# YQChen8/SSF-SLAM

Measured on AMD Instinct MI355X. Metric: LiDAR front-end frames/sec (mask+feature+GN), 64-beam 120k pts, 1/2/4/8 GPUs, higher is better.
Workload: dtype f32 features / f64 mask+solve

## Files before the change

ssf-slam_amd/csrc/mask_common.hpp:

```cpp
#pragma once
#include "ssf_device.hpp"
#include "ssf_internal.hpp"

#include <float.h>
#include <type_traits>

namespace ssf {

#ifndef SSF_MASK_THREADS
#define SSF_MASK_THREADS 768
#endif
constexpr int kMaskThreads = SSF_MASK_THREADS;

#ifdef SSF_MASK_STAMPS
#define SSF_STAMP(slot)                                                                   \
    do {                                                                                  \
        if (threadIdx.x == 0) {                                                           \
            const unsigned long long _t = __builtin_amdgcn_s_memtime();                   \
            out[26 + (slot)] = (double)(_t - stamp0);                                     \
        }                                                                                 \
    } while (0)
#else
#define SSF_STAMP(slot) do { } while (0)
#endif
constexpr int kNW = kMaskThreads / 64;
#ifndef SSF_LLOYD_DEEP
#define SSF_LLOYD_DEEP 2
#endif
constexpr int kLloydDeep = SSF_LLOYD_DEEP;
#ifndef SSF_KPP_DEEP
#define SSF_KPP_DEEP 2
#endif
constexpr int kKppBlocks = 4096;
constexpr double kPi = 3.14159265358979323846;
#ifndef SSF_LLOYD_FULL_PASSES
#define SSF_LLOYD_FULL_PASSES 4
#endif
constexpr int kLloydFullPasses = SSF_LLOYD_FULL_PASSES;
#ifndef SSF_LLOYD_REFULL
#define SSF_LLOYD_REFULL 4
#endif
constexpr int kLloydRefull = SSF_LLOYD_REFULL;
#ifndef SSF_LLOYD_REC_DEEP
#define SSF_LLOYD_REC_DEEP 8
#endif
constexpr int kLloydRecDeep = SSF_LLOYD_REC_DEEP;
constexpr int kLQ = SSF_LLOYD_REC_DEEP * 128;
constexpr int kLloydMax = 300;

SSF_DEV constexpr int up(int i, int j) { return i * 6 - (i * (i - 1)) / 2 + (j - i); }

struct MaskShared {
    double mean[6], tol;
    double tot[28];
    double cen[12], csn[2], cenp[12], csnp[2];
    double x0[6], ktot[16];
    double logdet[2], logw[2];
    double Aq[21], bq[6], cq, C0;
    double lb;
    double C[36], L[36];
    double sums[29];
    double lsum[14];
    double lhist[kLloydMax * 9];
    float lb1[512], lb2[512];
    int64_t c0, c1;
    double dg_cyc, dg_n, dg_lab, dg_wfull, dg_full1;
#ifdef SSF_MASK_STAMPS
    double dg_e[3];
#endif
    double passes;
    int km_iter, em_iter, strict, converged, done, status, label0, bg, bg_pred, lfull;
    double hnk[2], hq[2], hpm[12];
    int hrc[2];
};

template <class T>
SSF_DEV void load_x(const T* __restrict__ P, const T* __restrict__ Fl, int64_t i, double x[6]) {
    x[0] = (double)Fl[3 * i]; x[1] = (double)Fl[3 * i + 1]; x[2] = (double)Fl[3 * i + 2];
    x[3] = (double)P[3 * i];  x[4] = (double)P[3 * i + 1];  x[5] = (double)P[3 * i + 2];
}

typedef __attribute__((address_space(3))) const double LdsDouble;

SSF_DEV const LdsDouble* lds_laundered(const double* p) {
    uint32_t a = (uint32_t)(uintptr_t)p;
    asm volatile("" : "+v"(a));
    return (const LdsDouble*)(uintptr_t)a;
}

template <class T>
SSF_DEV void load_raw(const T* __restrict__ P, const T* __restrict__ Fl, int64_t i, T r[6]) {
    r[0] = Fl[3 * i]; r[1] = Fl[3 * i + 1]; r[2] = Fl[3 * i + 2];
    r[3] = P[3 * i];  r[4] = P[3 * i + 1];  r[5] = P[3 * i + 2];
}

#ifndef SSF_NT_POINTS
#define SSF_NT_POINTS 1
#endif
#if SSF_NT_POINTS
#define SSF_STREAM_LOAD(p) __builtin_nontemporal_load(p)
#else
#define SSF_STREAM_LOAD(p) (*(p))
#endif

template <class T>
SSF_DEV void load_raw_stream(const T* __restrict__ P, const T* __restrict__ Fl, int64_t i, T r[6]) {
    r[0] = SSF_STREAM_LOAD(&Fl[3 * i]); r[1] = SSF_STREAM_LOAD(&Fl[3 * i + 1]); r[2] = SSF_STREAM_LOAD(&Fl[3 * i + 2]);
    r[3] = SSF_STREAM_LOAD(&P[3 * i]);  r[4] = SSF_STREAM_LOAD(&P[3 * i + 1]);  r[5] = SSF_STREAM_LOAD(&P[3 * i + 2]);
}

template <class Ts>
SSF_DEV void load3_off(const Ts* __restrict__ base, uint32_t o, Ts r[3]) {
    const Ts* p = reinterpret_cast<const Ts*>(reinterpret_cast<const char*>(base) + o);
    r[0] = SSF_STREAM_LOAD(&p[0]); r[1] = SSF_STREAM_LOAD(&p[1]); r[2] = SSF_STREAM_LOAD(&p[2]);
}

SSF_DEV double uni(double v) {
    return __hiloint2double(__builtin_amdgcn_readfirstlane(__double2hiint(v)),
                            __builtin_amdgcn_readfirstlane(__double2loint(v)));
}

template <int D, class Ts, class Fn>
SSF_DEV void for_points_deep(const Ts* __restrict__ P, const Ts* __restrict__ Fl, int64_t r0, int64_t r1, Fn&& fn) {
    if (r1 <= r0) return;
    const Ts* Pb = P + 3 * r0;
    const Ts* Fb = Fl + 3 * r0;
    const uint32_t n = (uint32_t)(r1 - r0), T = blockDim.x, last = n - 1;
    constexpr uint32_t S = 3 * sizeof(Ts);
    const uint32_t j0 = threadIdx.x;
    auto load = [&](uint32_t k, Ts r[6]) { load3_off(Fb, k * S, r); load3_off(Pb, k * S, r + 3); };
    Ts buf[D][6];
#pragma unroll
    for (int d = 0; d < D; ++d) load(min(j0 + d * T, last), buf[d]);
    for (uint32_t base = j0; base < n; base += D * T) {
#pragma unroll
        for (int d = 0; d < D; ++d) {
            const uint32_t j = base + d * T;
            double x[6];
#pragma unroll
            for (int k = 0; k < 6; ++k) x[k] = (double)buf[d][k];
            load(min(j + D * T, last), buf[d]);
            fn(r0 + (int64_t)j, x, j < n);
        }
    }
}

template <class Ts, class Fn2, class Fn1>
SSF_DEV void for_point_pairs(const Ts* __restrict__ P, const Ts* __restrict__ Fl, int64_t r0, int64_t r1, Fn2&& fn2,
                             Fn1&& fn1) {
    const Ts* Pb = P + 3 * r0;
    const Ts* Fb = Fl + 3 * r0;
    const uint32_t n = (uint32_t)(r1 - r0), T = blockDim.x, last = n - 1;
    constexpr uint32_t S = 3 * sizeof(Ts);
    uint32_t i = threadIdx.x;
    if (i >= n) return;
    Ts ra[6], rb[6];
    auto load = [&](uint32_t k, Ts r[6]) { load3_off(Fb, k * S, r); load3_off(Pb, k * S, r + 3); };
    load(i, ra);
    load(min(i + T, last), rb);
    for (; i + T < n; i += 2 * T) {
        double xa[6], xb[6];
#pragma unroll
        for (int d = 0; d < 6; ++d) { xa[d] = (double)ra[d]; xb[d] = (double)rb[d]; }
        load(min(i + 2 * T, last), ra);
        load(min(i + 3 * T, last), rb);
        fn2(xa, xb);
    }
    if (i < n) {
        double xa[6];
#pragma unroll
        for (int d = 0; d < 6; ++d) xa[d] = (double)ra[d];
        fn1(xa);
    }
}

}
```

ssf-slam_amd/csrc/mask_lloyd.hpp:

```cpp
#pragma once
#include "mask_exchange.hpp"

namespace ssf {

SSF_DEV uint2* lloyd_rec_base(uint2* rec, int64_t fb, int f) {
    return rec + ((fb + kLloydSpareRecs * (int64_t)f + 1) & ~(int64_t)1);
}
SSF_DEV uint32_t* lloyd_queue_base(uint2* rec, int64_t total, int n_frames, int64_t fb, int f) {
    return reinterpret_cast<uint32_t*>(rec + lloyd_rec_count(total, n_frames)) + fb + kLloydSpareQueue * (int64_t)f;
}

template <class T>
SSF_DEV bool mask_lloyd(MaskCtx<T>& C, const MaskLds& L, uint2* __restrict__ lloyd_rec, int64_t total,
                        int n_frames) {
    MaskShared& S = L.S;
    const int tid = threadIdx.x;
    const T* P = C.P;
    const T* Fl = C.Fl;
    const double (&mean)[6] = C.mean;
    const int64_t n = C.n, r0 = C.X.r0, r1 = C.X.r1;
    if (tid == 0) { S.strict = 0; S.done = 0; S.lfull = 1; S.dg_cyc = S.dg_n = S.dg_lab = S.dg_wfull = S.dg_full1 = 0.0; }
    uint2* __restrict__ LR = lloyd_rec_base(lloyd_rec, C.fb, C.f);
    uint32_t* __restrict__ LQ = lloyd_queue_base(lloyd_rec, total, n_frames, C.fb, C.f);
    for (int it = 0; it < kLloydMax; ++it) {
        if (tid == 0) {
            double* h = S.lhist + 9 * it;
            for (int k = 0; k < 2; ++k) {
                double sn = 0.0;
                for (int d = 0; d < 6; ++d) sn += S.cen[6 * k + d] * S.cen[6 * k + d];
                S.csn[k] = sn;
            }
            for (int d = 0; d < 6; ++d) h[d] = S.cen[6 + d] - S.cen[d];
            h[6] = S.csn[0] - S.csn[1];
            h[7] = sqrt(S.csn[0]) + sqrt(S.csn[1]);
            h[8] = S.csn[0] + S.csn[1];
        }
        __syncthreads();
        if (tid < it) {
            const double* h = S.lhist + 9 * it;
            const double* g = S.lhist + 9 * tid;
            double dw = 0.0;
            for (int d = 0; d < 6; ++d) dw += (h[d] - g[d]) * (h[d] - g[d]);
            S.lb1[tid] = __double2float_ru(2.0 * sqrt(dw) + 2e-13 * (h[7] + g[7]));
            S.lb2[tid] = __double2float_ru(fabs(h[6] - g[6]) + 1e-13 * (h[8] + g[8]));
        }
        __syncthreads();
        const double csn0 = uni(S.csn[0]), csn1 = uni(S.csn[1]);
        double acc[14];
#pragma unroll
        for (int k = 0; k < 14; ++k) acc[k] = 0.0;
        int changed = 0, nlab = 0;
        const bool full = S.lfull != 0;
#ifdef SSF_MASK_STAMPS
        const unsigned long long pass_t0 = __builtin_amdgcn_s_memtime();
#endif
        const bool wrec = it >= kLloydFullPasses - 1;
        auto label = [&](auto wrec_c, int64_t i, const double* x, int lp, bool val) {
            const LdsDouble* cen = lds_laundered(S.cen);
            double v[6], dt0 = 0.0, dt1 = 0.0, vn = 0.0;
#pragma unroll
            for (int d = 0; d < 6; ++d) {
                v[d] = x[d] - mean[d];
                dt0 += v[d] * cen[d]; dt1 += v[d] * cen[6 + d]; vn += v[d] * v[d];
            }
            const double D0 = -2.0 * dt0 + csn0, D1 = -2.0 * dt1 + csn1;
            const int l = D1 < D0 ? 1 : 0;
            double d1 = full ? (double)l : (double)(l - lp), d0 = full ? 1.0 - d1 : -d1;
            d1 = val ? d1 : 0.0; d0 = val ? d0 : 0.0;
            changed += val && (it == 0 || l != lp);
            acc[0] += d0; acc[7] += d1;
#pragma unroll
            for (int d = 0; d < 6; ++d) { acc[1 + d] += d0 * v[d]; acc[8 + d] += d1 * v[d]; }
            const uint32_t gb = __float_as_uint((float)fabs(D0 - D1));
            const uint32_t nvb = (__float_as_uint(__builtin_sqrtf((float)vn)) + 4u + 0x1FFu) & 0x7FFFFE00u;
            if constexpr (decltype(wrec_c)::value) LR[val ? i : n] = make_uint2(gb ? gb - 1u : 0u, nvb | (uint32_t)it | ((uint32_t)l << 31));
        };
        if (full) {
            const double cpn0 = uni(S.csnp[0]), cpn1 = uni(S.csnp[1]);
            auto full_pass = [&](auto wrec_c) {
                for_points_deep<kLloydDeep>(P, Fl, r0, r1, [&](int64_t i, const double* x, bool val) {
                    const LdsDouble* cenp = lds_laundered(S.cenp);
                    double dp0 = 0.0, dp1 = 0.0;
#pragma unroll
                    for (int d = 0; d < 6; ++d) {
                        const double v = x[d] - mean[d];
                        dp0 += v * cenp[d]; dp1 += v * cenp[6 + d];
                    }
                    const int lp = (-2.0 * dp1 + cpn1) < (-2.0 * dp0 + cpn0) ? 1 : 0;
                    label(wrec_c, i, x, lp, val);
                });
            };
            if (wrec) full_pass(std::true_type{});
            else full_pass(std::false_type{});
            nlab = (int)((r1 - r0 - tid + blockDim.x - 1) / blockDim.x);
        } else {
            const int w = __builtin_amdgcn_readfirstlane(tid >> 6), lane = lane_id();
            const int64_t seg = ((r1 - r0 + kNW - 1) / kNW + 127) / 128 * 128;
            const int64_t ws = r0 + (int64_t)w * seg, we = ws + seg < r1 ? ws + seg : r1;
            uint32_t* __restrict__ WQ = LQ + ws;
            const int64_t qspare = n - ws;
            const uint4* __restrict__ LR4 = reinterpret_cast<const uint4*>(LR);
            const int64_t plast = (n - 1) >> 1;
            uint32_t* Q = L.lq + w * kLQ;
            int qc = 0, nl = 0;
            constexpr int D = kLloydRecDeep;
            uint4 buf[D];
#pragma unroll
            for (int d = 0; d < D; ++d) buf[d] = LR4[min((ws >> 1) + d * 64 + lane, plast)];
            for (int64_t base = ws; base < we; base += D * 128) {
#pragma unroll
                for (int d = 0; d < D; ++d) {
                    const int64_t b = base + d * 128;
                    const uint4 q = buf[d];
#pragma unroll
                    for (int h = 0; h < 2; ++h) {
                        const uint32_t gx = h ? q.z : q.x, gy = h ? q.w : q.y;
                        const int64_t i = b + 2 * lane + h;
                        const int tr = (int)(gy & 0x1FFu);
                        const float nv = __uint_as_float(gy & 0x7FFFFE00u);
                        const bool skip = __uint_as_float(gx) > __builtin_fmaf(S.lb1[tr], nv, S.lb2[tr]) * 1.00001f;
                        const bool nd = (i < we) & !skip;
                        const uint64_t m = __ballot(nd);
                        if (nd) Q[nl + __popcll(m & lanemask_lt())] = (uint32_t)i | (gy & 0x80000000u);
                        nl += __popcll(m);
                    }
                    buf[d] = LR4[min(((b + D * 128) >> 1) + lane, plast)];
                }
                __builtin_amdgcn_wave_barrier();
#pragma unroll
                for (int h = 0; h < 2; ++h)
                    WQ[h * 64 + lane < nl ? qc + h * 64 + lane : qspare + lane] = Q[h * 64 + lane];
                for (int k = 128; k < nl; k += 64)
                    if (k + lane < nl) WQ[qc + k + lane] = Q[k + lane];
                __builtin_amdgcn_wave_barrier();
                qc += nl;
                nl = 0;
            }
            __threadfence_block();
            for (int j0 = 0; j0 < qc; j0 += 512) {
                uint32_t e[8];
#pragma unroll
                for (int k = 0; k < 8; ++k) e[k] = WQ[min(j0 + k * 64 + lane, qc - 1)];
                T px[8][6];
#pragma unroll
                for (int k = 0; k < 8; ++k) load_raw(P, Fl, (int64_t)(e[k] & 0x7FFFFFFFu), px[k]);
#pragma unroll
                for (int k = 0; k < 8; ++k) {
                    double x[6];
#pragma unroll
                    for (int d = 0; d < 6; ++d) x[d] = (double)px[k][d];
                    const bool val = j0 + k * 64 + lane < qc;
                    label(std::true_type{}, (int64_t)(e[k] & 0x7FFFFFFFu), x, (int)(e[k] >> 31), val);
                    nlab += val ? 1 : 0;
                }
            }
        }
        block_sum_rs<14>(acc, L.red);
        changed = block_sum_scalar<int>(changed, L.ired);
        nlab = block_sum_scalar<int>(nlab, L.ired);
        if (C.X.G > 1) {
            double v[16];
#pragma unroll
            for (int k = 0; k < 14; ++k) v[k] = acc[k];
            v[14] = (double)changed; v[15] = (double)nlab;
            if (!exchange<16>(C.X, v, L.xtmp, &L.okflag)) return false;
#pragma unroll
            for (int k = 0; k < 14; ++k) acc[k] = v[k];
            changed = (int)v[14]; nlab = (int)v[15];
        }
        if (tid == 0) {
            S.passes += full ? 1.0 + (wrec ? 8.0 / 24.0 : 0.0)
                             : (8.0 * (double)n + 40.0 * (double)nlab) / (24.0 * (double)n);
            S.km_iter = it + 1;
            for (int k = 0; k < 14; ++k) S.lsum[k] = full ? acc[k] : S.lsum[k] + acc[k];
            S.lfull = full ? it < kLloydFullPasses - 1 : nlab * kLloydRefull > n;
#ifdef SSF_MASK_STAMPS
            if (!full) { S.dg_cyc += (double)(__builtin_amdgcn_s_memtime() - pass_t0); S.dg_n += 1.0; S.dg_lab += nlab; }
            else if (it == kLloydFullPasses - 1) S.dg_wfull = (double)(__builtin_amdgcn_s_memtime() - pass_t0);
            else if (it == 1) S.dg_full1 = (double)(__builtin_amdgcn_s_memtime() - pass_t0);
#endif
            for (int k = 0; k < 12; ++k) S.cenp[k] = S.cen[k];
            S.csnp[0] = S.csn[0]; S.csnp[1] = S.csn[1];
            double shift = 0.0;
            for (int k = 0; k < 2; ++k) {
                const double wgt = S.lsum[7 * k];
                double sh = 0.0;
                for (int d = 0; d < 6; ++d) {
                    const double nc = wgt > 0.0 ? S.lsum[7 * k + 1 + d] * (1.0 / wgt) : S.cen[6 * k + d];
                    const double df = nc - S.cen[6 * k + d];
                    sh += df * df;
                    S.cen[6 * k + d] = nc;
                }
                sh = sqrt(sh);
                shift += sh * sh;
            }
            if (changed == 0) { S.strict = 1; S.done = 1; }
            else if (shift <= S.tol) S.done = 1;
        }
        __syncthreads();
        if (S.done) break;
    }
    return true;
}

}
```

ssf-slam_amd/csrc/mask_seed.hpp:

```cpp
#pragma once
#include "mask_exchange.hpp"

namespace ssf {

template <class T>
SSF_DEV bool mask_pass0(MaskCtx<T>& C, const MaskLds& L, const double* __restrict__ draws) {
    MaskShared& S = L.S;
    const int tid = threadIdx.x;
    const T* P = C.P;
    const T* Fl = C.Fl;
    const int64_t n = C.n, r0 = C.X.r0, r1 = C.X.r1;
    double x0[6];
    load_x(P, Fl, 0, x0);
    double a[27];
#pragma unroll
    for (int i = 0; i < 27; ++i) a[i] = 0.0;
    for_points_deep<kLloydDeep>(P, Fl, r0, r1, [&](int64_t, const double* x, bool val) {
        double v[6], vw[6];
#pragma unroll
        for (int d = 0; d < 6; ++d) { v[d] = x[d] - x0[d]; vw[d] = val ? v[d] : 0.0; a[d] += vw[d]; }
#pragma unroll
        for (int r = 0; r < 6; ++r)
#pragma unroll
            for (int c = r; c < 6; ++c) a[6 + up(r, c)] += vw[r] * v[c];
    });
    block_sum_rs<27>(a, L.red);
    if (!exchange<27>(C.X, a, L.xtmp, &L.okflag)) return false;
    if (tid == 0) {
        const double nn = (double)n;
        double m[6];
        double tol = 0.0;
        for (int d = 0; d < 6; ++d) { m[d] = a[d] / nn; S.mean[d] = x0[d] + m[d]; }
        S.tot[0] = nn;
        for (int d = 0; d < 6; ++d) S.tot[1 + d] = a[d] - nn * m[d];
        for (int r = 0; r < 6; ++r)
            for (int c = r; c < 6; ++c) S.tot[7 + up(r, c)] = a[6 + up(r, c)] - nn * m[r] * m[c];
        for (int d = 0; d < 6; ++d) tol += S.tot[7 + up(d, d)] / nn;
        S.tol = tol / 6.0 * 1e-4;
        for (int d = 0; d < 6; ++d) S.x0[d] = x0[d];
        S.ktot[0] = nn;
        for (int r = 0; r < 3; ++r) { S.ktot[1 + r] = a[r] + a[3 + r]; S.ktot[4 + r] = a[3 + r]; }
        for (int r = 0; r < 3; ++r)
            for (int c = 0; c < 3; ++c) {
                const int fr = r, pr = 3 + r, pc = 3 + c;
                const double sfp = a[6 + (fr <= pc ? up(fr, pc) : up(pc, fr))];
                const double spp = a[6 + (pr <= pc ? up(pr, pc) : up(pc, pr))];
                S.ktot[7 + r * 3 + c] = sfp + spp;
            }
        S.c0 = (int64_t)draws[3 * C.f];
        if (S.c0 < 0) S.c0 = 0;
        if (S.c0 >= n) S.c0 = n - 1;
        S.passes = 1;
    }
    __syncthreads();
    return true;
}

template <class T>
SSF_DEV bool mask_kmeanspp(MaskCtx<T>& C, const MaskLds& L, const double* __restrict__ draws) {
    MaskShared& S = L.S;
    const int tid = threadIdx.x;
    const T* P = C.P;
    const T* Fl = C.Fl;
    const double (&mean)[6] = C.mean;
    const int64_t n = C.n, r0 = C.X.r0, r1 = C.X.r1;
    const int f = C.f;
    double c0[6], cn0 = 0.0;
    {
        double x[6];
        load_x(P, Fl, S.c0, x);
        for (int d = 0; d < 6; ++d) { c0[d] = x[d] - mean[d]; cn0 += c0[d] * c0[d]; }
    }
    const int nw = blockDim.x >> 6, w = tid >> 6, lane = lane_id();
    const int64_t nloc = r1 - r0;
    const int64_t seg = (((nloc + nw - 1) / nw) + 63) / 64 * 64;
    const int64_t ws = r0 + (int64_t)w * seg, we = ws + seg < r1 ? ws + seg : r1;
    auto dist0x = [&](const double* x) {
        double dt = 0.0, xs = 0.0;
#pragma unroll
        for (int d = 0; d < 6; ++d) { const double v = x[d] - mean[d]; dt += c0[d] * v; xs += v * v; }
        const double v = (-2.0 * dt + cn0) + xs;
        return v > 0.0 ? v : 0.0;
    };
    auto dist0 = [&](int64_t i) {
        double x[6];
        load_x(P, Fl, i, x);
        return dist0x(x);
    };
    constexpr int kKppDeep = SSF_KPP_DEEP;
    const int64_t wlast = we > ws ? we - 1 : ws;
    const int64_t spw = seg / 64;
    const bool use_blocks = spw * nw <= kKppBlocks;
    double wsum = 0.0;
    T kb[kKppDeep][6];
    if (ws < we) {
#pragma unroll
        for (int k = 0; k < kKppDeep; ++k) load_raw_stream(P, Fl, min(ws + 64 * k + lane, wlast), kb[k]);
    }
    for (int64_t b0 = ws; b0 < we; b0 += 64 * kKppDeep)
#pragma unroll
    for (int k = 0; k < kKppDeep; ++k) {
        const int64_t b = b0 + 64 * k;
        if (b >= we) break;
        const int64_t i = b + lane;
        double x[6];
#pragma unroll
        for (int d = 0; d < 6; ++d) x[d] = (double)kb[k][d];
        load_raw_stream(P, Fl, min(i + 64 * kKppDeep, wlast), kb[k]);
        const double d = i < we ? dist0x(x) : 0.0;
        wsum += d;
        if (use_blocks) {
            double v = d;
#pragma unroll
            for (int o = 1; o < 64; o <<= 1) {
                const double y = __shfl_up(v, o, 64);
                if (lane >= o) v += y;
            }
            if (lane == 63) L.bsum[w * spw + (b - ws) / 64] = v;
        }
    }
    wsum = wave_sum(wsum);
    if (lane == 0) L.red[w] = wsum;
    if (tid == 0) { L.cand[0] = (unsigned long long)n; L.cand[1] = (unsigned long long)n; }
    __syncthreads();
    double pot = 0.0, carry = 0.0;
    for (int k = 0; k < nw; ++k) { if (k == w) carry = pot; pot += L.red[k]; }
    if (C.X.G > 1) {
        double before = 0.0, total = 0.0;
        if (!exchange_prefix(C.X, pot, L.xtmp, &L.okflag, before, total)) return false;
        carry += before;
        pot = total;
    }
    if (tid == 0) S.passes += 1;
    const double t1 = draws[3 * f + 1] * pot, t2 = draws[3 * f + 2] * pot;
    const double wtot = L.red[w];
    bool f1 = carry + wtot < t1 * (1.0 - 1e-9), f2 = carry + wtot < t2 * (1.0 - 1e-9);
    if (use_blocks) {
        int64_t blk1 = -1, blk2 = -1;
        double cb1 = 0.0, cb2 = 0.0;
        if (lane == 0 && !(f1 && f2)) {
            double cr = carry;
            for (int64_t k = 0; ws + 64 * k < we; ++k) {
                const double tot = L.bsum[w * spw + k];
                if (!f1 && blk1 < 0 && cr + tot >= t1) { blk1 = k; cb1 = cr; }
                if (!f2 && blk2 < 0 && cr + tot >= t2) { blk2 = k; cb2 = cr; }
                if ((f1 || blk1 >= 0) && (f2 || blk2 >= 0)) break;
                cr += tot;
            }
        }
        blk1 = __shfl(blk1, 0, 64); blk2 = __shfl(blk2, 0, 64);
        cb1 = __shfl(cb1, 0, 64); cb2 = __shfl(cb2, 0, 64);
#pragma unroll
        for (int j = 0; j < 2; ++j) {
            const int64_t blk = j ? blk2 : blk1;
            if (blk < 0) continue;
            const int64_t b = ws + 64 * blk;
            const int64_t i = b + lane;
            double v = i < we ? dist0(i) : 0.0;
#pragma unroll
            for (int o = 1; o < 64; o <<= 1) {
                const double y = __shfl_up(v, o, 64);
                if (lane >= o) v += y;
            }
            const double incl = (j ? cb2 : cb1) + v;
            const uint64_t mm = __ballot(i < we && incl >= (j ? t2 : t1));
            if (mm && lane == 0) atomicMin(&L.cand[j], (unsigned long long)(b + __ffsll((unsigned long long)mm) - 1));
        }
        f1 = f2 = true;
    }
    for (int64_t b = ws; b < we && !(f1 && f2); b += 64) {
        const int64_t i = b + lane;
        double v = i < we ? dist0(i) : 0.0;
#pragma unroll
        for (int o = 1; o < 64; o <<= 1) {
            const double y = __shfl_up(v, o, 64);
            if (lane >= o) v += y;
        }
        const double incl = carry + v;
        const uint64_t m1 = __ballot(i < we && incl >= t1), m2 = __ballot(i < we && incl >= t2);
        if (!f1 && m1) { f1 = true; if (lane == 0) atomicMin(&L.cand[0], (unsigned long long)(b + __ffsll((unsigned long long)m1) - 1)); }
        if (!f2 && m2) { f2 = true; if (lane == 0) atomicMin(&L.cand[1], (unsigned long long)(b + __ffsll((unsigned long long)m2) - 1)); }
        carry += __shfl(v, 63, 64);
    }
    __syncthreads();
    double cmin[2] = {(double)L.cand[0], (double)L.cand[1]};
    if (!exchange<2, true>(C.X, cmin, L.xtmp, &L.okflag)) return false;
    const int64_t cand[2] = {cmin[0] < (double)n ? (int64_t)cmin[0] : n - 1,
                             cmin[1] < (double)n ? (int64_t)cmin[1] : n - 1};
    double cc[2][6], ccn[2] = {0.0, 0.0};
    for (int j = 0; j < 2; ++j) {
        double x[6];
        load_x(P, Fl, cand[j], x);
        for (int d = 0; d < 6; ++d) { cc[j][d] = x[d] - mean[d]; ccn[j] += cc[j][d] * cc[j][d]; }
    }
    double cp[2] = {0.0, 0.0};
    if (ws < we) {
#pragma unroll
        for (int k = 0; k < kKppDeep; ++k) load_raw_stream(P, Fl, min(ws + 64 * k + lane, wlast), kb[k]);
    }
    for (int64_t b0 = ws; b0 < we; b0 += 64 * kKppDeep)
#pragma unroll
    for (int k = 0; k < kKppDeep; ++k) {
        const int64_t b = b0 + 64 * k;
        if (b >= we) break;
        const int64_t i = b + lane;
        double x[6];
#pragma unroll
        for (int d = 0; d < 6; ++d) x[d] = (double)kb[k][d];
        load_raw_stream(P, Fl, min(i + 64 * kKppDeep, wlast), kb[k]);
        if (i < we) {
            double xs = 0.0, dt0 = 0.0, dt1 = 0.0, dtc = 0.0;
#pragma unroll
            for (int d = 0; d < 6; ++d) {
                const double v = x[d] - mean[d];
                dtc += c0[d] * v; xs += v * v; dt0 += cc[0][d] * v; dt1 += cc[1][d] * v;
            }
            double di = (-2.0 * dtc + cn0) + xs;
            di = di > 0.0 ? di : 0.0;
            double v0 = (-2.0 * dt0 + ccn[0]) + xs, v1 = (-2.0 * dt1 + ccn[1]) + xs;
            v0 = v0 > 0.0 ? v0 : 0.0; v1 = v1 > 0.0 ? v1 : 0.0;
            cp[0] += v0 < di ? v0 : di;
            cp[1] += v1 < di ? v1 : di;
        }
    }
    block_sum<2>(cp, L.red);
    if (!exchange<2>(C.X, cp, L.xtmp, &L.okflag)) return false;
    if (tid == 0) {
        const int best = cp[1] < cp[0] ? 1 : 0;
        S.c1 = cand[best];
        for (int d = 0; d < 6; ++d) { S.cen[d] = c0[d]; S.cen[6 + d] = cc[best][d]; }
        for (int d = 0; d < 12; ++d) S.cenp[d] = 0.0;
        S.csnp[0] = S.csnp[1] = 0.0;
        S.passes += 2;
    }
    __syncthreads();
    return true;
}

}
```

Before: 65600.

## Fuse k-means++ distance prefix into pass0 and first Lloyd step into candidate pass

The per-block prefix sums of distance to the first centre now come from the moments pass (pass0), so k-means++ no longer rereads all points to build them. The final candidate-evaluation sweep also accumulates the Lloyd iteration-0 assignment sums for both candidate centres. It then keeps the winning set and performs the first centroid update, so Lloyd starts at iteration 1. This removes two full streaming passes over the point cloud, at the cost of more registers and a wider reduction (30 values) in the fused loops.

After: 68550 (median of 6 runs). 4.5% higher.

```diff
diff --git a/ssf-slam_amd/csrc/mask_common.hpp b/ssf-slam_amd/csrc/mask_common.hpp
--- a/ssf-slam_amd/csrc/mask_common.hpp
+++ b/ssf-slam_amd/csrc/mask_common.hpp
@@ -120,7 +120,7 @@
                             __builtin_amdgcn_readfirstlane(__double2loint(v)));
 }
 
-template <int D, class Ts, class Fn>
+template <int D, bool kWaveTrips = false, class Ts, class Fn>
 SSF_DEV void for_points_deep(const Ts* __restrict__ P, const Ts* __restrict__ Fl, int64_t r0, int64_t r1, Fn&& fn) {
     if (r1 <= r0) return;
     const Ts* Pb = P + 3 * r0;
@@ -128,11 +128,12 @@
     const uint32_t n = (uint32_t)(r1 - r0), T = blockDim.x, last = n - 1;
     constexpr uint32_t S = 3 * sizeof(Ts);
     const uint32_t j0 = threadIdx.x;
+    const uint32_t lead = kWaveTrips ? (j0 & 63u) : 0u;
     auto load = [&](uint32_t k, Ts r[6]) { load3_off(Fb, k * S, r); load3_off(Pb, k * S, r + 3); };
     Ts buf[D][6];
 #pragma unroll
     for (int d = 0; d < D; ++d) load(min(j0 + d * T, last), buf[d]);
-    for (uint32_t base = j0; base < n; base += D * T) {
+    for (uint32_t base = j0; base - lead < n; base += D * T) {
 #pragma unroll
         for (int d = 0; d < D; ++d) {
             const uint32_t j = base + d * T;
diff --git a/ssf-slam_amd/csrc/mask_lloyd.hpp b/ssf-slam_amd/csrc/mask_lloyd.hpp
--- a/ssf-slam_amd/csrc/mask_lloyd.hpp
+++ b/ssf-slam_amd/csrc/mask_lloyd.hpp
@@ -8,6 +8,47 @@
 }
 SSF_DEV uint32_t* lloyd_queue_base(uint2* rec, int64_t total, int n_frames, int64_t fb, int f) {
     return reinterpret_cast<uint32_t*>(rec + lloyd_rec_count(total, n_frames)) + fb + kLloydSpareQueue * (int64_t)f;
+}
+
+SSF_DEV void lloyd_reset(MaskShared& S) {
+    S.strict = 0; S.done = 0; S.lfull = 1;
+    S.dg_cyc = S.dg_n = S.dg_lab = S.dg_wfull = S.dg_full1 = 0.0;
+}
+SSF_DEV void lloyd_begin_pass(MaskShared& S, int it) {
+    double* h = S.lhist + 9 * it;
+    for (int k = 0; k < 2; ++k) {
+        double sn = 0.0;
+        for (int d = 0; d < 6; ++d) sn += S.cen[6 * k + d] * S.cen[6 * k + d];
+        S.csn[k] = sn;
+    }
+    for (int d = 0; d < 6; ++d) h[d] = S.cen[6 + d] - S.cen[d];
+    h[6] = S.csn[0] - S.csn[1];
+    h[7] = sqrt(S.csn[0]) + sqrt(S.csn[1]);
+    h[8] = S.csn[0] + S.csn[1];
+}
+SSF_DEV void lloyd_end_pass(MaskShared& S, int it, bool full, const double (&acc)[14], int changed, int nlab,
+                            int64_t n, double cost) {
+    S.passes += cost;
+    S.km_iter = it + 1;
+    for (int k = 0; k < 14; ++k) S.lsum[k] = full ? acc[k] : S.lsum[k] + acc[k];
+    S.lfull = full ? it < kLloydFullPasses - 1 : nlab * kLloydRefull > n;
+    for (int k = 0; k < 12; ++k) S.cenp[k] = S.cen[k];
+    S.csnp[0] = S.csn[0]; S.csnp[1] = S.csn[1];
+    double shift = 0.0;
+    for (int k = 0; k < 2; ++k) {
+        const double wgt = S.lsum[7 * k];
+        double sh = 0.0;
+        for (int d = 0; d < 6; ++d) {
+            const double nc = wgt > 0.0 ? S.lsum[7 * k + 1 + d] * (1.0 / wgt) : S.cen[6 * k + d];
+            const double df = nc - S.cen[6 * k + d];
+            sh += df * df;
+            S.cen[6 * k + d] = nc;
+        }
+        sh = sqrt(sh);
+        shift += sh * sh;
+    }
+    if (changed == 0) { S.strict = 1; S.done = 1; }
+    else if (shift <= S.tol) S.done = 1;
 }
 
 template <class T>
@@ -19,22 +60,12 @@
     const T* Fl = C.Fl;
     const double (&mean)[6] = C.mean;
     const int64_t n = C.n, r0 = C.X.r0, r1 = C.X.r1;
-    if (tid == 0) { S.strict = 0; S.done = 0; S.lfull = 1; S.dg_cyc = S.dg_n = S.dg_lab = S.dg_wfull = S.dg_full1 = 0.0; }
+    static_assert(kLloydFullPasses >= 2, "iteration 0 (mask_kmeanspp) writes no records");
+    if (S.done) return true;
     uint2* __restrict__ LR = lloyd_rec_base(lloyd_rec, C.fb, C.f);
     uint32_t* __restrict__ LQ = lloyd_queue_base(lloyd_rec, total, n_frames, C.fb, C.f);
-    for (int it = 0; it < kLloydMax; ++it) {
-        if (tid == 0) {
-            double* h = S.lhist + 9 * it;
-            for (int k = 0; k < 2; ++k) {
-                double sn = 0.0;
-                for (int d = 0; d < 6; ++d) sn += S.cen[6 * k + d] * S.cen[6 * k + d];
-                S.csn[k] = sn;
-            }
-            for (int d = 0; d < 6; ++d) h[d] = S.cen[6 + d] - S.cen[d];
-            h[6] = S.csn[0] - S.csn[1];
-            h[7] = sqrt(S.csn[0]) + sqrt(S.csn[1]);
-            h[8] = S.csn[0] + S.csn[1];
-        }
+    for (int it = 1; it < kLloydMax; ++it) {
+        if (tid == 0) lloyd_begin_pass(S, it);
         __syncthreads();
         if (tid < it) {
             const double* h = S.lhist + 9 * it;
@@ -169,33 +200,14 @@
             changed = (int)v[14]; nlab = (int)v[15];
         }
         if (tid == 0) {
-            S.passes += full ? 1.0 + (wrec ? 8.0 / 24.0 : 0.0)
-                             : (8.0 * (double)n + 40.0 * (double)nlab) / (24.0 * (double)n);
-            S.km_iter = it + 1;
-            for (int k = 0; k < 14; ++k) S.lsum[k] = full ? acc[k] : S.lsum[k] + acc[k];
-            S.lfull = full ? it < kLloydFullPasses - 1 : nlab * kLloydRefull > n;
+            lloyd_end_pass(S, it, full, acc, changed, nlab, n,
+                           full ? 1.0 + (wrec ? 8.0 / 24.0 : 0.0)
+                                : (8.0 * (double)n + 40.0 * (double)nlab) / (24.0 * (double)n));
 #ifdef SSF_MASK_STAMPS
             if (!full) { S.dg_cyc += (double)(__builtin_amdgcn_s_memtime() - pass_t0); S.dg_n += 1.0; S.dg_lab += nlab; }
             else if (it == kLloydFullPasses - 1) S.dg_wfull = (double)(__builtin_amdgcn_s_memtime() - pass_t0);
             else if (it == 1) S.dg_full1 = (double)(__builtin_amdgcn_s_memtime() - pass_t0);
 #endif
-            for (int k = 0; k < 12; ++k) S.cenp[k] = S.cen[k];
-            S.csnp[0] = S.csn[0]; S.csnp[1] = S.csn[1];
-            double shift = 0.0;
-            for (int k = 0; k < 2; ++k) {
-                const double wgt = S.lsum[7 * k];
-                double sh = 0.0;
-                for (int d = 0; d < 6; ++d) {
-                    const double nc = wgt > 0.0 ? S.lsum[7 * k + 1 + d] * (1.0 / wgt) : S.cen[6 * k + d];
-                    const double df = nc - S.cen[6 * k + d];
-                    sh += df * df;
-                    S.cen[6 * k + d] = nc;
-                }
-                sh = sqrt(sh);
-                shift += sh * sh;
-            }
-            if (changed == 0) { S.strict = 1; S.done = 1; }
-            else if (shift <= S.tol) S.done = 1;
         }
         __syncthreads();
         if (S.done) break;
diff --git a/ssf-slam_amd/csrc/mask_seed.hpp b/ssf-slam_amd/csrc/mask_seed.hpp
--- a/ssf-slam_amd/csrc/mask_seed.hpp
+++ b/ssf-slam_amd/csrc/mask_seed.hpp
@@ -1,7 +1,43 @@
 #pragma once
-#include "mask_exchange.hpp"
+#include "mask_lloyd.hpp"
 
 namespace ssf {
+
+SSF_DEV double dist0(const double* x, const double (&xc)[6]) {
+    double s = 0.0;
+#pragma unroll
+    for (int d = 0; d < 6; ++d) { const double u = x[d] - xc[d]; s += u * u; }
+    return s;
+}
+
+SSF_DEV int64_t first_centre(const double* __restrict__ draws, int f, int64_t n) {
+    int64_t c0 = (int64_t)draws[3 * f];
+    if (c0 < 0) c0 = 0;
+    if (c0 >= n) c0 = n - 1;
+    return c0;
+}
+
+struct KppSeg {
+    int64_t seg, spw;
+    bool use_blocks;
+};
+SSF_DEV KppSeg kpp_seg(int64_t nloc) {
+    KppSeg k;
+    const int nw = blockDim.x >> 6;
+    k.seg = (((nloc + nw - 1) / nw) + 63) / 64 * 64;
+    k.spw = k.seg / 64;
+    k.use_blocks = k.spw * nw <= kKppBlocks;
+    return k;
+}
+
+SSF_DEV double block_scan(double v, int lane) {
+#pragma unroll
+    for (int o = 1; o < 64; o <<= 1) {
+        const double y = __shfl_up(v, o, 64);
+        if (lane >= o) v += y;
+    }
+    return v;
+}
 
 template <class T>
 SSF_DEV bool mask_pass0(MaskCtx<T>& C, const MaskLds& L, const double* __restrict__ draws) {
@@ -10,12 +46,14 @@
     const T* P = C.P;
     const T* Fl = C.Fl;
     const int64_t n = C.n, r0 = C.X.r0, r1 = C.X.r1;
-    double x0[6];
+    double x0[6], xc0[6];
     load_x(P, Fl, 0, x0);
+    const int64_t c0 = first_centre(draws, C.f, n);
+    load_x(P, Fl, c0, xc0);
     double a[27];
 #pragma unroll
     for (int i = 0; i < 27; ++i) a[i] = 0.0;
-    for_points_deep<kLloydDeep>(P, Fl, r0, r1, [&](int64_t, const double* x, bool val) {
+    auto moments = [&](const double* x, bool val) {
         double v[6], vw[6];
 #pragma unroll
         for (int d = 0; d < 6; ++d) { v[d] = x[d] - x0[d]; vw[d] = val ? v[d] : 0.0; a[d] += vw[d]; }
@@ -23,7 +61,19 @@
         for (int r = 0; r < 6; ++r)
 #pragma unroll
             for (int c = r; c < 6; ++c) a[6 + up(r, c)] += vw[r] * v[c];
-    });
+    };
+    if (kpp_seg(r1 - r0).use_blocks) {
+        const int lane = lane_id();
+        const uint32_t nblk = (uint32_t)((r1 - r0 + 63) >> 6);
+        for_points_deep<kLloydDeep, true>(P, Fl, r0, r1, [&](int64_t i, const double* x, bool val) {
+            moments(x, val);
+            const double d = block_scan(val ? dist0(x, xc0) : 0.0, lane);
+            const uint32_t blk = (uint32_t)(i - r0) >> 6;
+            if (lane == 63 && blk < nblk) L.bsum[blk] = d;
+        });
+    } else {
+        for_points_deep<kLloydDeep>(P, Fl, r0, r1, [&](int64_t, const double* x, bool val) { moments(x, val); });
+    }
     block_sum_rs<27>(a, L.red);
     if (!exchange<27>(C.X, a, L.xtmp, &L.okflag)) return false;
     if (tid == 0) {
@@ -47,9 +97,7 @@
                 const double spp = a[6 + (pr <= pc ? up(pr, pc) : up(pc, pr))];
                 S.ktot[7 + r * 3 + c] = sfp + spp;
             }
-        S.c0 = (int64_t)draws[3 * C.f];
-        if (S.c0 < 0) S.c0 = 0;
-        if (S.c0 >= n) S.c0 = n - 1;
+        S.c0 = c0;
         S.passes = 1;
     }
     __syncthreads();
@@ -65,59 +113,43 @@
     const double (&mean)[6] = C.mean;
     const int64_t n = C.n, r0 = C.X.r0, r1 = C.X.r1;
     const int f = C.f;
-    double c0[6], cn0 = 0.0;
-    {
-        double x[6];
-        load_x(P, Fl, S.c0, x);
-        for (int d = 0; d < 6; ++d) { c0[d] = x[d] - mean[d]; cn0 += c0[d] * c0[d]; }
-    }
+    double xc0[6], c0[6], cn0 = 0.0;
+    load_x(P, Fl, S.c0, xc0);
+    for (int d = 0; d < 6; ++d) { c0[d] = xc0[d] - mean[d]; cn0 += c0[d] * c0[d]; }
     const int nw = blockDim.x >> 6, w = tid >> 6, lane = lane_id();
-    const int64_t nloc = r1 - r0;
-    const int64_t seg = (((nloc + nw - 1) / nw) + 63) / 64 * 64;
+    const KppSeg ks = kpp_seg(r1 - r0);
+    const int64_t seg = ks.seg, spw = ks.spw;
+    const bool use_blocks = ks.use_blocks;
     const int64_t ws = r0 + (int64_t)w * seg, we = ws + seg < r1 ? ws + seg : r1;
-    auto dist0x = [&](const double* x) {
-        double dt = 0.0, xs = 0.0;
-#pragma unroll
-        for (int d = 0; d < 6; ++d) { const double v = x[d] - mean[d]; dt += c0[d] * v; xs += v * v; }
-        const double v = (-2.0 * dt + cn0) + xs;
-        return v > 0.0 ? v : 0.0;
-    };
-    auto dist0 = [&](int64_t i) {
+    auto dist0i = [&](int64_t i) {
         double x[6];
         load_x(P, Fl, i, x);
-        return dist0x(x);
+        return dist0(x, xc0);
     };
     constexpr int kKppDeep = SSF_KPP_DEEP;
     const int64_t wlast = we > ws ? we - 1 : ws;
-    const int64_t spw = seg / 64;
-    const bool use_blocks = spw * nw <= kKppBlocks;
     double wsum = 0.0;
-    T kb[kKppDeep][6];
-    if (ws < we) {
-#pragma unroll
-        for (int k = 0; k < kKppDeep; ++k) load_raw_stream(P, Fl, min(ws + 64 * k + lane, wlast), kb[k]);
-    }
-    for (int64_t b0 = ws; b0 < we; b0 += 64 * kKppDeep)
-#pragma unroll
-    for (int k = 0; k < kKppDeep; ++k) {
-        const int64_t b = b0 + 64 * k;
-        if (b >= we) break;
-        const int64_t i = b + lane;
-        double x[6];
-#pragma unroll
-        for (int d = 0; d < 6; ++d) x[d] = (double)kb[k][d];
-        load_raw_stream(P, Fl, min(i + 64 * kKppDeep, wlast), kb[k]);
-        const double d = i < we ? dist0x(x) : 0.0;
-        wsum += d;
-        if (use_blocks) {
-            double v = d;
-#pragma unroll
-            for (int o = 1; o < 64; o <<= 1) {
-                const double y = __shfl_up(v, o, 64);
-                if (lane >= o) v += y;
-            }
-            if (lane == 63) L.bsum[w * spw + (b - ws) / 64] = v;
-        }
+    if (use_blocks) {
+        for (int64_t k = lane; ws + 64 * k < we; k += 64) wsum += L.bsum[w * spw + k];
+    } else {
+        T kb[kKppDeep][6];
+        if (ws < we) {
+#pragma unroll
+            for (int k = 0; k < kKppDeep; ++k) load_raw_stream(P, Fl, min(ws + 64 * k + lane, wlast), kb[k]);
+        }
+        for (int64_t b0 = ws; b0 < we; b0 += 64 * kKppDeep)
+#pragma unroll
+        for (int k = 0; k < kKppDeep; ++k) {
+            const int64_t b = b0 + 64 * k;
+            if (b >= we) break;
+            const int64_t i = b + lane;
+            double x[6];
+#pragma unroll
+            for (int d = 0; d < 6; ++d) x[d] = (double)kb[k][d];
+            load_raw_stream(P, Fl, min(i + 64 * kKppDeep, wlast), kb[k]);
+            wsum += i < we ? dist0(x, xc0) : 0.0;
+        }
+        if (tid == 0) S.passes += 1;
     }
     wsum = wave_sum(wsum);
     if (lane == 0) L.red[w] = wsum;
@@ -131,7 +163,6 @@
         carry += before;
         pot = total;
     }
-    if (tid == 0) S.passes += 1;
     const double t1 = draws[3 * f + 1] * pot, t2 = draws[3 * f + 2] * pot;
     const double wtot = L.red[w];
     bool f1 = carry + wtot < t1 * (1.0 - 1e-9), f2 = carry + wtot < t2 * (1.0 - 1e-9);
@@ -156,26 +187,18 @@
             if (blk < 0) continue;
             const int64_t b = ws + 64 * blk;
             const int64_t i = b + lane;
-            double v = i < we ? dist0(i) : 0.0;
-#pragma unroll
-            for (int o = 1; o < 64; o <<= 1) {
-                const double y = __shfl_up(v, o, 64);
-                if (lane >= o) v += y;
-            }
+            const double v = block_scan(i < we ? dist0i(i) : 0.0, lane);
             const double incl = (j ? cb2 : cb1) + v;
             const uint64_t mm = __ballot(i < we && incl >= (j ? t2 : t1));
             if (mm && lane == 0) atomicMin(&L.cand[j], (unsigned long long)(b + __ffsll((unsigned long long)mm) - 1));
         }
         f1 = f2 = true;
+    } else if (tid == 0) {
+        S.passes += 1;
     }
     for (int64_t b = ws; b < we && !(f1 && f2); b += 64) {
         const int64_t i = b + lane;
-        double v = i < we ? dist0(i) : 0.0;
-#pragma unroll
-        for (int o = 1; o < 64; o <<= 1) {
-            const double y = __shfl_up(v, o, 64);
-            if (lane >= o) v += y;
-        }
+        const double v = block_scan(i < we ? dist0i(i) : 0.0, lane);
         const double incl = carry + v;
         const uint64_t m1 = __ballot(i < we && incl >= t1), m2 = __ballot(i < we && incl >= t2);
         if (!f1 && m1) { f1 = true; if (lane == 0) atomicMin(&L.cand[0], (unsigned long long)(b + __ffsll((unsigned long long)m1) - 1)); }
@@ -193,45 +216,50 @@
         load_x(P, Fl, cand[j], x);
         for (int d = 0; d < 6; ++d) { cc[j][d] = x[d] - mean[d]; ccn[j] += cc[j][d] * cc[j][d]; }
     }
-    double cp[2] = {0.0, 0.0};
-    if (ws < we) {
-#pragma unroll
-        for (int k = 0; k < kKppDeep; ++k) load_raw_stream(P, Fl, min(ws + 64 * k + lane, wlast), kb[k]);
-    }
-    for (int64_t b0 = ws; b0 < we; b0 += 64 * kKppDeep)
-#pragma unroll
-    for (int k = 0; k < kKppDeep; ++k) {
-        const int64_t b = b0 + 64 * k;
-        if (b >= we) break;
-        const int64_t i = b + lane;
-        double x[6];
-#pragma unroll
-        for (int d = 0; d < 6; ++d) x[d] = (double)kb[k][d];
-        load_raw_stream(P, Fl, min(i + 64 * kKppDeep, wlast), kb[k]);
-        if (i < we) {
-            double xs = 0.0, dt0 = 0.0, dt1 = 0.0, dtc = 0.0;
-#pragma unroll
-            for (int d = 0; d < 6; ++d) {
-                const double v = x[d] - mean[d];
-                dtc += c0[d] * v; xs += v * v; dt0 += cc[0][d] * v; dt1 += cc[1][d] * v;
-            }
-            double di = (-2.0 * dtc + cn0) + xs;
-            di = di > 0.0 ? di : 0.0;
-            double v0 = (-2.0 * dt0 + ccn[0]) + xs, v1 = (-2.0 * dt1 + ccn[1]) + xs;
-            v0 = v0 > 0.0 ? v0 : 0.0; v1 = v1 > 0.0 ? v1 : 0.0;
-            cp[0] += v0 < di ? v0 : di;
-            cp[1] += v1 < di ? v1 : di;
-        }
-    }
-    block_sum<2>(cp, L.red);
-    if (!exchange<2>(C.X, cp, L.xtmp, &L.okflag)) return false;
+    double s[30];
+#pragma unroll
+    for (int k = 0; k < 30; ++k) s[k] = 0.0;
+    int one_hi;
+    asm volatile("s_mov_b32 %0, 0x3ff00000" : "=s"(one_hi));
+    const double one = __hiloint2double(one_hi, 0);
+    for_points_deep<kLloydDeep>(P, Fl, r0, r1, [&](int64_t, const double* x, bool val) {
+        double v[6], dtc = 0.0, dt[2] = {0.0, 0.0}, xs = 0.0;
+#pragma unroll
+        for (int d = 0; d < 6; ++d) {
+            v[d] = x[d] - mean[d];
+            dtc += v[d] * c0[d]; dt[0] += v[d] * cc[0][d]; dt[1] += v[d] * cc[1][d]; xs += v[d] * v[d];
+        }
+        const double di = dist0(x, xc0);
+        const double D0 = -2.0 * dtc + cn0;
+#pragma unroll
+        for (int j = 0; j < 2; ++j) {
+            const double D1 = -2.0 * dt[j] + ccn[j];
+            double vj = D1 + xs;
+            vj = vj > 0.0 ? vj : 0.0;
+            vj = vj < di ? vj : di;
+            s[j] += val ? vj : 0.0;
+            double d1 = D1 < D0 ? one : 0.0, d0 = 1.0 - d1;
+            d1 = val ? d1 : 0.0; d0 = val ? d0 : 0.0;
+            double* acc = s + 2 + 14 * j;
+            acc[0] += d0; acc[7] += d1;
+#pragma unroll
+            for (int d = 0; d < 6; ++d) { acc[1 + d] += d0 * v[d]; acc[8 + d] += d1 * v[d]; }
+        }
+    });
+    block_sum_rs<30>(s, L.red);
+    if (!exchange<30>(C.X, s, L.xtmp, &L.okflag)) return false;
+    const bool best = s[1] < s[0];
+    double acc[14];
+#pragma unroll
+    for (int k = 0; k < 14; ++k) acc[k] = best ? s[16 + k] : s[2 + k];
     if (tid == 0) {
-        const int best = cp[1] < cp[0] ? 1 : 0;
-        S.c1 = cand[best];
-        for (int d = 0; d < 6; ++d) { S.cen[d] = c0[d]; S.cen[6 + d] = cc[best][d]; }
+        S.c1 = cand[best ? 1 : 0];
+        for (int d = 0; d < 6; ++d) { S.cen[d] = c0[d]; S.cen[6 + d] = best ? cc[1][d] : cc[0][d]; }
         for (int d = 0; d < 12; ++d) S.cenp[d] = 0.0;
         S.csnp[0] = S.csnp[1] = 0.0;
-        S.passes += 2;
+        lloyd_reset(S);
+        lloyd_begin_pass(S, 0);
+        lloyd_end_pass(S, 0, true, acc, n > 0x7fffffff ? 0x7fffffff : (int)n, 0, n, 1.0);
     }
     __syncthreads();
     return true;
```
